# INP-PM/FEDM

Measured on AMD Instinct MI355X. Metric: BDF2 DOF-updates/sec (streamer_discharge 2D axisym), higher is better.
Workload: dtype f64

## Files before the change

### __graft_entry__.py

```python
import os
import subprocess
import sys
from pathlib import Path

ROOT = Path(__file__).resolve().parent
CSRC = ROOT / "fedm_amd" / "csrc"
LIB = ROOT / "fedm_amd" / "libfedm_hip.so"
SOURCES = ["prep.cpp", "kernels.hip", "assemble.hip", "boundary.hip", "spmv.hip", "assemble3.hip", "gd.hip", "gdprep.hip", "amg.hip", "fs_tiles.hip",
           "segregated.hip", "comm.hip", "photo.hip", "diag.hip", "fields.hip", "gd_balance.hip", "gd_fields.hip", "currents.hip", "context.cpp", "photo_abi.cpp", "krylov.cpp", "newton.cpp", "amg_setup.cpp", "hooks.cpp"]
HEADERS = [CSRC / "fedm_internal.hpp", CSRC / "element.hpp", CSRC / "element_lean.hpp", CSRC / "amg.hpp",
           CSRC / "comm.hpp", CSRC / "species_planes.hpp", CSRC / "solver.hpp", CSRC / "device_util.hpp", CSRC / "table_lookup.h", CSRC / "photo.hpp", CSRC / "diag.hpp", CSRC / "fields.hpp", CSRC / "gd_balance.hpp", CSRC / "currents.hpp",
           CSRC / "postproc.hpp", ROOT / "include" / "fedm_hip.h"]


OBJ = CSRC / "_build"
FILE_FLAGS = {"assemble3.hip": ["-mllvm", "-disable-machine-licm"]}


def _stale(lib):
    if not Path(lib).exists():
        return True
    t = Path(lib).stat().st_mtime
    return any(p.stat().st_mtime > t for p in [CSRC / s for s in SOURCES] + HEADERS)


def _compile(hipcc, src, obj, extra):
    cmd = [hipcc, "--offload-arch=gfx950", "-O3", "-std=c++17", "-fPIC", "-c", "-Wno-unused-result",
           "-Wno-unused-value", f"-I{ROOT / 'include'}", f"-I{CSRC}", *FILE_FLAGS.get(Path(src).name, []), *extra,
           "-o", str(obj), str(src)]
    subprocess.run(cmd, check=True)


def build(force=False, lib=LIB, defines=()):
    if force or _stale(lib):
        import fcntl
# ... 101 lines not shown
```

### fedm_amd/_lib.py

```python
import ctypes as C
import os
from pathlib import Path

MAX_SPECIES, MAX_TERMS, MAX_REACTIONS, MAX_TAGS = 4, 6, 8, 8
MAX_QP, MAX_FQP, MAX_EXT_NODES = 32, 8, 10
MAX_TABLES, MAX_TABLE_KNOTS = 16, 4096

EQ_TYPES = {"reaction": 0, "diffusion-reaction": 1, "drift-diffusion-reaction": 2}
BC_KINDS = {"zero flux": 0, "Neumann": 1, "flux source": 2}
DIVERGED = {1: "maximum number of Newton iterations reached",
            2: "NaN or Inf in the residual", 3: "linear solve (GMRES) did not converge"}


class TermSumC(C.Structure):
    _fields_ = [("n_terms", C.c_int32), ("pad_", C.c_int32),
                ("c", C.c_double * MAX_TERMS), ("p", C.c_double * MAX_TERMS),
                ("q", C.c_double * MAX_TERMS), ("r", C.c_double * MAX_TERMS)]


class ModelDesc(C.Structure):
    _fields_ = [
        ("n_species", C.c_int32), ("poisson", C.c_int32), ("axisymmetric", C.c_int32),
        ("n_reactions", C.c_int32),
        ("eq_type", C.c_int32 * MAX_SPECIES), ("Z", C.c_double * MAX_SPECIES),
# ... 57 lines not shown
class MeshDesc(C.Structure):
    _fields_ = [("n_vertices", C.c_int32), ("n_cells", C.c_int32),
                ("coords", C.POINTER(C.c_double)), ("cells", C.POINTER(C.c_int32)),
                ("facet_tags", C.POINTER(C.c_int8)),
                ("n_dirichlet", C.c_int32),
                ("dirichlet_dofs", C.POINTER(C.c_int32)),
                ("dirichlet_vals", C.POINTER(C.c_double)),
                ("n_owned_vertices", C.c_int32),
                ("n_identity_vertices", C.c_int32), ("identity_vertices", C.POINTER(C.c_int32)),
                ("halo_depth", C.c_int32)]


class NewtonOpts(C.Structure):
    _fields_ = [("rtol", C.c_double), ("atol", C.c_double), ("stol", C.c_double),
                ("max_it", C.c_int32), ("ksp_restart", C.c_int32),
                ("ksp_rtol", C.c_double), ("ksp_atol", C.c_double),
                ("ksp_max_it", C.c_int32), ("watch_component", C.c_int32)]


class NewtonReport(C.Structure):
    _fields_ = [("iterations", C.c_int32), ("converged", C.c_int32),
                ("linear_iterations", C.c_int32), ("reason", C.c_int32),
                ("fnorm0", C.c_double), ("fnorm", C.c_double)]


class Csr(C.Structure):
    _fields_ = [("n_rows", C.c_int32), ("n_cols", C.c_int32),
                ("indptr", C.POINTER(C.c_int64)), ("indices", C.POINTER(C.c_int32)),
                ("values", C.POINTER(C.c_double))]


PHOTO_MAX_TERMS = 4


class PhotoDesc(C.Structure):
    _fields_ = [("n_terms", C.c_int32), ("n_src", C.c_int32),
                ("c", C.c_double * PHOTO_MAX_TERMS), ("kappa", C.c_double * PHOTO_MAX_TERMS),
                ("efficiency", C.c_double), ("src_reaction", C.c_int32 * MAX_REACTIONS),
                ("target_species_mask", C.c_uint32), ("zero_tag_mask", C.c_uint32)]


class PhotoHierarchy(C.Structure):
    _fields_ = [("n_levels", C.c_int32), ("nu", C.c_int32),
                ("A", C.POINTER(Csr)), ("P", C.POINTER(Csr)), ("R", C.POINTER(Csr)),
                ("coarse_inverse", C.POINTER(C.c_double)), ("omega", C.c_double)]

# ... 93 lines not shown
    "fedm_debug_gd_reduced_field": (C.c_int, [_P, _D]),
    "fedm_gd_update_mean_energy": (C.c_int, [_P]),
    "fedm_get_state_old": (C.c_int, [_P, _D]),
    "fedm_ctx_destroy": (None, [_P]),
    "fedm_set_state": (C.c_int, [_P, _D, _D, _D]),
    "fedm_get_state": (C.c_int, [_P, _D]),
    "fedm_shift_state": (C.c_int, [_P]),
    "fedm_reset_state": (C.c_int, [_P]),
    "fedm_state_snapshot": (C.c_int, [_P]),
    "fedm_state_restore": (C.c_int, [_P]),
    "fedm_set_step": (C.c_int, [_P, C.c_double, C.c_double]),
    "fedm_set_dirichlet_values": (C.c_int, [_P, _D]),
    "fedm_set_ext_source": (C.c_int, [_P, C.c_int, _D]),
    "fedm_ext_source_program": (C.c_int, [_P, C.c_int, C.c_int, C.POINTER(C.c_int32), C.c_int, _D, C.c_int]),
    "fedm_ext_source_eval": (C.c_int, [_P, C.c_int, _D]),
    "fedm_debug_get_ext_source": (C.c_int, [_P, C.c_int, _D]),
    "fedm_residual": (C.c_int, [_P, _D, _D]),
    "fedm_jacobian": (C.c_int, [_P]),
    "fedm_jacobian_nnz": (C.c_int64, [_P]),
    "fedm_jacobian_csr": (C.c_int, [_P, C.POINTER(C.c_int64), C.POINTER(C.c_int32), _D]),
    "fedm_spmv": (C.c_int, [_P, _D, _D]),
    "fedm_newton_solve": (C.c_int, [_P, C.POINTER(NewtonOpts), C.POINTER(NewtonReport)]),
    "fedm_poisson_solve": (C.c_int, [_P, C.c_double, C.c_int, C.POINTER(C.c_int)]),
    "fedm_poisson_update": (C.c_int, [_P, C.c_double, C.c_int, C.POINTER(C.c_int)]),
    "fedm_newton_solve_species": (C.c_int, [_P, C.POINTER(NewtonOpts), C.POINTER(NewtonReport)]),
    "fedm_segregated_stats": (C.c_int, [_P, C.POINTER(C.c_int64), C.c_int]),
    "fedm_debug_species_assembly": (C.c_int, [_P, C.c_int]),
    "fedm_debug_block_product": (C.c_int, [_P, C.c_int, _D, _D]),
    "fedm_debug_species_linear_solve": (C.c_int, [_P, _D, C.POINTER(NewtonOpts), _D, C.POINTER(C.c_int), _D]),
    "fedm_photo_setup": (C.c_int, [_P, C.POINTER(PhotoDesc), C.POINTER(PhotoHierarchy)]),
    "fedm_photo_update": (C.c_int, [_P, C.c_double, C.c_int, C.POINTER(C.c_int)]),
    "fedm_photo_get": (C.c_int, [_P, _D, _D]),
    "fedm_photo_stats": (C.c_int, [_P, C.POINTER(C.c_int64), C.c_int]),
    "fedm_diag_setup": (C.c_int, [_P, _D, C.POINTER(C.c_int8), C.c_int]),
    "fedm_diagnostics": (C.c_int, [_P, C.POINTER(DiagOpts), C.POINTER(DiagOut)]),
    "fedm_gd_balance_setup": (C.c_int, [_P, _D, C.POINTER(C.c_int8), C.c_int]),
    "fedm_gd_balance": (C.c_int, [_P, C.POINTER(GdBalanceOut)]),
    "fedm_currents_setup": (C.c_int, [_P, C.c_int, _D]),
    "fedm_currents_solve": (C.c_int, [_P, C.POINTER(PhotoHierarchy), _D, C.c_double, C.c_int, C.POINTER(C.c_int)]),
    "fedm_currents_get_psi": (C.c_int, [_P, _D]),
    "fedm_currents": (C.c_int, [_P, C.POINTER(CurrentsOut)]),
    "fedm_fields_setup": (C.c_int, [_P, C.POINTER(Csr)]),
    "fedm_probe_setup": (C.c_int, [_P, C.c_int, C.POINTER(C.c_int32), _D]),
    "fedm_fields": (C.c_int, [_P, C.POINTER(FieldOpts), C.c_int, C.POINTER(FieldReq), _D, _D, C.POINTER(C.c_int32),
                              C.POINTER(C.c_int32)]),
    "fedm_gd_fields_setup": (C.c_int, [_P, C.POINTER(Csr)]),
# ... 109 lines not shown
```

### fedm_amd/cases/streamer.py

```python
from pathlib import Path

import numpy as np

from ..device import DeviceProblem, Model, Reaction
from ..mesh import Marking_boundaries, Mesh, RectangleMesh, geometric_lines
from ..termsum import TermSum, parse

U_W = 18750.0
BOX = 0.0125
BOUNDARIES = [["line", 0.0, 0.0, 0.0, BOX], ["line", BOX, BOX, 0.0, BOX],
              ["line", 0.0, BOX, 0.0, 0.0], ["line", 0.0, BOX, BOX, BOX]]
BC_TYPE = [["zero flux", "Neumann"], ["zero flux", "Neumann"],
           ["zero flux", "zero flux"], ["zero flux", "zero flux"]]
DECK = Path(__file__).resolve().parents[2] / "decks" / "streamer_discharge" / "file_input"
MU_E = "2.3987*E_m**(-0.26)"
D_E = "4.3628e-3*E_m**(0.22)"
ALPHA = "(1.1944e6 + 4.3666e26 * E_m**(-3))*exp(-2.73e7/E_m)-340.75"
N0 = 760.0 * 3.21877e22


def model(mu_e=MU_E, D_e=D_E, alpha=ALPHA, quadrature_degree=2):
    mu = parse(mu_e)
    rate = parse(alpha) * mu * TermSum.field()
    return Model(n_species=2, poisson=True,
# ... 100 lines not shown

SPECIES_NAMES = ("ions", "electrons")

DIAGNOSTIC_COLUMNS = ("t", "z_head", "E_max_axis", "E_max", "N_i", "N_e", "net_charge", "surface_charge_cathode",
                      "surface_charge_anode", "current", "ni_max", "ne_max")


MULTIGRID = dict(nu=1, omega=0.85, hard_poly_degree=2)


def initialise(prob, multigrid=True):
    U = np.zeros((prob.nv, 3))
    U[:, 0], U[:, 1] = initial_log_densities(prob.coords)
    prob.set_state(U, U, U)
    if multigrid:
        prob.setup_multigrid(**MULTIGRID)
        from ..device import chebyshev_weights
        prob.set_fieldsplit(chebyshev_weights(6), hard_weights=chebyshev_weights(4))
    its = prob.poisson_solve(rtol=1e-12)
    U = prob.get_state()
    prob.set_state(U, U, U)
    return U, its



class Stepper:

    partition_name = "single GPU"

    @property
    def assembly_kernel_name(self):
        sz = self.prob.sizes()
        if sz["assembly_variant"] == "lds-patches/one-pass":
            return (f"assemble_lean3_kernel<2,1,{sz['patch_threads']},kept planes> (LDS patches with micro-coloured cell "
                    "order, one pass over the cells, live planes only, F+J)")
        if sz["assembly_variant"] != "lds-patches":
            return f"volume assembly, variant '{sz['assembly_variant']}' (F+J)"
        return (f"assemble_lean2_kernel<2,1,{sz['patch_threads']}> (LDS patches with micro-coloured cell order, one "
                "equation row at a time, F+J)")

    @property
    def multigrid_levels(self):
        return getattr(self.prob, "multigrid_levels", None)

    def __init__(self, prob, dt_init=5e-12, dt_max=5e-12, dt_min=1e-15, ttol=1e-3,
                 relative_tolerance=1e-4, maximum_iterations=20, error_file=None, quiet=True,
                 coupling="coupled"):
        import tempfile
        from .. import functions as ff
        from ..forms import DeviceState, Expression, FunctionAssigner
        self.ff, self.prob = ff, prob
        self.solver = ff.PETScSNESSolver()
        self.solver.parameters["relative_tolerance"] = relative_tolerance
        self.solver.parameters["maximum_iterations"] = maximum_iterations
        self.solver.parameters["coupling"] = coupling
        self.problem = ff.Problem(None, None, [], device_problem=prob)
        self.dt = Expression("time_step", time_step=dt_init, degree=0)
        self.dt_old = Expression("time_step", time_step=1e30, degree=0)
        self.u_new, self.u_old = DeviceState(prob, "new"), DeviceState(prob, "old")
        self.assigner = FunctionAssigner()
        self.error, self.max_error = [0.0] * 2, [1] * 3
        self.ttol, self.dt_min, self.dt_max = ttol, dt_min, dt_max
        if error_file is None:
            error_file = Path(tempfile.mkdtemp(prefix="fedm_amd_")) / "relative error.log"
        self.error_file = Path(error_file)
        open(self.error_file, "w").close()
        self.t, self.steps, self.newton_iterations, self.linear_iterations = 0.0, 0, 0, 0
        self.quiet = quiet
        self.total_dofs = prob.n

    def initialise(self):
        return initialise(self.prob)

    def step(self):
        import contextlib, io
        ff = self.ff
        self.prob.shift_state()
        sink = io.StringIO() if self.quiet else None
        with (contextlib.redirect_stdout(sink) if sink else contextlib.nullcontext()):
            self.t = ff.adaptive_solver(self.solver, self.problem, self.t, self.dt, self.dt_old,
                                        self.u_new, self.u_old, None, None, self.assigner,
                                        self.error, self.error_file, self.max_error, self.ttol,
                                        self.dt_min, time_dependent_arguments=[],
                                        approximation="LFA")
        self.newton_iterations += self.prob.last_report.iterations
        self.linear_iterations += self.prob.last_report.linear_iterations
        self.dt_old.time_step = self.dt.time_step
        self.dt.time_step = ff.adaptive_timestep(self.dt.time_step, self.max_error, self.ttol,
                                                 self.dt_min, self.dt_max)
        self.max_error[2] = self.max_error[1]
        self.max_error[1] = self.max_error[0]
        self.steps += 1
        return self.t

    def diagnose(self):
        if getattr(self, "_diagnose", None) is None:
            self._diagnose = diagnostics(self.prob)
# ... 61 lines not shown
```

### fedm_amd/csrc/context.cpp

```cpp
#include <algorithm>
#include <cmath>
#include <cstdlib>
#include <cstring>

#include "photo.hpp"
#include "solver.hpp"

namespace fedm {

static thread_local std::string g_error;
void set_error(const std::string &msg) { g_error = msg; }

void prof_collect(Ctx &c) {
    Prof &p = c.prof;
    if (p.used == 0) return;
    hipStreamSynchronize(c.stream);
    for (int i = 0; i + 1 < p.used; i += 2) {
        float ms = 0.f;
        if (hipEventElapsedTime(&ms, p.ev[i], p.ev[i + 1]) == hipSuccess) {
            p.ms[p.kind[i / 2]] += ms;
            p.cnt[p.kind[i / 2]]++;
        }
    }
    p.used = 0;
// ... 205 lines not shown
        std::memcpy(buf.data() + sizeof(m) + sizeof(mt), t.x, sizeof(double) * total);
        std::memcpy(buf.data() + sizeof(m) + sizeof(mt) + sizeof(double) * total, t.y, sizeof(double) * total);
    }
    FEDM_HIP_CHECK(hipMalloc((void **)&dst, buf.size()));
    FEDM_HIP_CHECK(hipMemcpy(dst, buf.data(), buf.size(), hipMemcpyHostToDevice));
    return 0;
}

int put_vec(Ctx &c, double *dst, const double *src) {
    if (!src) return 0;
    std::memcpy(c.h_stage, src, sizeof(double) * c.n);
    FEDM_HIP_CHECK(hipMemcpyAsync(dst, c.h_stage, sizeof(double) * c.n, hipMemcpyHostToDevice, c.stream));
    FEDM_HIP_CHECK(hipStreamSynchronize(c.stream));
    return 0;
}

int get_vec(Ctx &c, double *dst, const double *src) {
    FEDM_HIP_CHECK(hipMemcpyAsync(c.h_stage, src, sizeof(double) * c.n, hipMemcpyDeviceToHost, c.stream));
    FEDM_HIP_CHECK(hipStreamSynchronize(c.stream));
    std::memcpy(dst, c.h_stage, sizeof(double) * c.n);
    return 0;
}

}

using namespace fedm;

extern "C" {

const char *fedm_last_error(void) { return g_error.c_str(); }
int fedm_abi_version(void) { return FEDM_ABI_VERSION; }

static int ctx_create_impl(const fedm_mesh_desc *mesh, const fedm_model_desc *model,
                           const fedm_gd_desc *gd, const HostTables &tables, int device, fedm_ctx **out);

static int ctx_create_guarded(const fedm_mesh_desc *mesh, const fedm_model_desc *model,
                              const fedm_gd_desc *gd, const HostTables &tables, int device, fedm_ctx **out) {
    *out = nullptr;
    fedm_ctx *h = nullptr;
    const int rc = ctx_create_impl(mesh, model, gd, tables, device, &h);
    if (rc != 0) {
        const std::string msg = g_error;
        if (h) fedm_ctx_destroy(h);
        g_error = msg;
        return rc;
    }
// ... 467 lines not shown
int fedm_set_state(fedm_ctx *h, const double *u_new, const double *u_old, const double *u_old1) {
    Ctx &c = h->c;
    c.err_cache_comp = -1;
    FEDM_HIP_CHECK(hipSetDevice(c.device));
    if (u_new) c.halo_pending = false;
    if (put_vec(c, c.d_u, u_new) || put_vec(c, c.d_uold, u_old) || put_vec(c, c.d_uold1, u_old1)) return -1;
    return 0;
}

int fedm_get_state(fedm_ctx *h, double *u_new) {
    Ctx &c = h->c;
    FEDM_HIP_CHECK(hipSetDevice(c.device));
    return get_vec(c, u_new, c.d_u);
}

int fedm_get_state_old(fedm_ctx *h, double *u_old) {
    Ctx &c = h->c;
    FEDM_HIP_CHECK(hipSetDevice(c.device));
    return get_vec(c, u_old, c.d_uold);
}

int fedm_shift_state(fedm_ctx *h) {
    Ctx &c = h->c;
    c.err_cache_comp = -1;
    FEDM_HIP_CHECK(hipSetDevice(c.device));
    std::swap(c.d_uold1, c.d_uold);
    launch_scale_copy(c, 1.0, c.d_u, c.d_uold);
    return 0;
}

int fedm_reset_state(fedm_ctx *h) {
    Ctx &c = h->c;
    c.err_cache_comp = -1;
    FEDM_HIP_CHECK(hipSetDevice(c.device));
    launch_scale_copy(c, 1.0, c.d_uold, c.d_u);
    return 0;
}

int fedm_state_snapshot(fedm_ctx *h) {
    Ctx &c = h->c;
    FEDM_HIP_CHECK(hipSetDevice(c.device));
    if (c.halo_pending) {
        comm_halo(c, c.d_u);
        c.halo_pending = false;
    }
    if (!c.d_snapshot) FEDM_HIP_CHECK(hipMalloc((void **)&c.d_snapshot, sizeof(double) * 3 * c.np));
    const double *src[3] = {c.d_u, c.d_uold, c.d_uold1};
    for (int k = 0; k < 3; ++k)
        FEDM_HIP_CHECK(hipMemcpyAsync(c.d_snapshot + (size_t)k * c.np, src[k], sizeof(double) * c.np,
                                      hipMemcpyDeviceToDevice, c.stream));
    FEDM_HIP_CHECK(hipStreamSynchronize(c.stream));
    c.snap_krylov_steps_hint = c.krylov_steps_hint;
    std::copy(std::begin(c.krylov_hints), std::end(c.krylov_hints), std::begin(c.snap_krylov_hints));
    c.snap_newton_its_hint = c.newton_its_hint;
    return 0;
}

int fedm_state_restore(fedm_ctx *h) {
// ... 297 lines not shown
```

### fedm_amd/csrc/newton.cpp

```cpp
#include <chrono>
#include <cmath>

#include "solver.hpp"

namespace fedm {

void set_hard_mode(Ctx &c, bool hard) {
    if (c.fs_alt_active == hard) return;
    c.fs_skip_sample = true;
    hipStreamSynchronize(c.stream);
    iter_graphs_clear(c);
    c.fs_alt_active = hard;
    if (c.fs_alt_sweeps > 0) {
        c.fs_sweeps = hard ? c.fs_alt_sweeps : c.fs_main_sweeps;
        for (int i = 0; i < c.fs_sweeps; ++i) c.fs_w[i] = hard ? c.fs_alt_w[i] : c.fs_main_w[i];
    }
    if (c.amg_alt) std::swap(c.amg, c.amg_alt);
}

static void update_fieldsplit_policy(Ctx &c, int it, int lin_total, int rc,
                                     std::chrono::steady_clock::time_point t_begin) {
    ++c.fs_solves[c.fs_alt_active ? 1 : 0];
    if ((c.fs_alt_sweeps > 0 || c.amg_alt) && it > 0) {
        const double per_solve = (double)lin_total / it;
// ... 149 lines not shown
                    indices[pos] = col * neq + cc;
                    values[pos] = val[(bc * neq2 + cr * neq + cc) * SLICE + l];
                    ++pos;
                }
            }
            indptr[(size_t)v * neq + cr + 1] = pos;
        }
    }
    return 0;
}

int fedm_spmv(fedm_ctx *h, const double *x, double *y) {
    Ctx &c = h->c;
    FEDM_HIP_CHECK(hipSetDevice(c.device));
    FEDM_HIP_CHECK(hipMemsetAsync(c.d_tmp, 0, sizeof(double) * c.np, c.stream));
    if (put_vec(c, c.d_tmp, x)) return -1;
    launch_spmv(c, c.d_tmp, c.d_w, false);
    return get_vec(c, y, c.d_w);
}

int fedm_newton_solve(fedm_ctx *h, const fedm_newton_opts *o, fedm_newton_report *rep) {
    Ctx &c = h->c;
    FEDM_HIP_CHECK(hipSetDevice(c.device));
    c.err_cache_comp = -1;
    const auto t_begin = std::chrono::steady_clock::now();
    int it = 0, lin_total = 0, rc = 0;
    double fnorm = 0.0, fnorm0 = 0.0, snorm = 0.0, xnorm = 0.0;
    while (true) {
        const bool residual_only = it > 0 && it == c.newton_its_hint;
        if (residual_only) {
            launch_assemble(c, false, 0);
            launch_finalize(c, false, 0);
        } else {
            eval_jacobian(c, 0);
        }
        const bool sums_local = c.comm && it > 0 && c.red12_local;
        const bool with_error = residual_only && (!c.comm || sums_local) && o->watch_component > 0 &&
                                o->watch_component <= c.neq;
        if (with_error) launch_field_error_slots34(c, o->watch_component - 1);
        norm2_publish(c, c.d_F, 0, with_error ? 5 : 3, sums_local ? (with_error ? 5 : 3) : 1);
        c.red12_local = false;
        bool planes_done = false;
        if (!residual_only && right_preconditioned(c)) {
            prepare_preconditioner_and_rhs(c);
            planes_done = true;
        }
// ... 45 lines not shown
        }
        if (c.comm && c.assembly_overlap) c.halo_pending = true;
        else comm_halo(c, c.d_u);
        if (comm_failed(c)) {
            rc = -1;
            break;
        }
        ++it;
    }
    if (comm_failed(c)) rc = -1;
    if (rc == 0) c.newton_its_hint = it;
    update_fieldsplit_policy(c, it, lin_total, rc, t_begin);
    write_report(rep, it, lin_total, fnorm0, fnorm, rc);
    if (comm_failed(c)) {
        set_error(c.comm->error);
        return -1;
    }
    if (hipGetLastError() != hipSuccess) {
        set_error("HIP error during Newton solve");
        return -1;
    }
    return rc;
}

int fedm_poisson_solve(fedm_ctx *h, double rtol, int max_it, int *iterations) {
    Ctx &c = h->c;
    c.err_cache_comp = -1;
    FEDM_HIP_CHECK(hipSetDevice(c.device));
    if (!c.poisson) {
        set_error("model has no Poisson row");
        return -2;
    }
    launch_set_dirichlet_state(c);
    launch_assemble(c, true, 1);
    launch_finalize(c, true, 1);
    launch_block_inverse(c);
    launch_scale_copy(c, -1.0, c.d_F, c.d_rhs);
    if (ensure_krylov(c, 1)) return -1;
    const CgResult cg = preconditioned_cg(c, CgMatrix::whole, rtol, max_it);
    launch_axpy(c, 1.0, c.d_V, c.d_u);
    comm_halo(c, c.d_u);
    FEDM_HIP_CHECK(hipStreamSynchronize(c.stream));
    if (iterations) *iterations = cg.it;
    if (comm_failed(c)) {
        set_error(c.comm->error);
        return -1;
// ... 84 lines not shown
    } else {
        launch_assemble(c, false, 0);
        launch_finalize(c, false, 0);
    }
    launch_pick_entries(c, 1, -1.0, c.d_F, c.d_rhs);
    if (ensure_krylov(c, 1)) return -1;
    const CgResult cg = preconditioned_cg(c, CgMatrix::potential_block, rtol, max_it);
    if (std::isfinite(cg.rn)) launch_axpy(c, 1.0, c.d_V, c.d_u);
    FEDM_HIP_CHECK(hipStreamSynchronize(c.stream));
    FEDM_HIP_CHECK(hipGetLastError());
    c.seg_stats[SG_CG_ITS] += cg.it;
    if (iterations) *iterations = cg.it;
    if (!std::isfinite(cg.rn)) return FEDM_DIVERGED_NAN;
    return cg.rn <= rtol * cg.r0 ? 0 : FEDM_DIVERGED_LINEAR;
}

int fedm_field_error(fedm_ctx *h, int component, double *rel_err) {
    Ctx &c = h->c;
    if (component < 0 || component >= c.neq) {
        set_error("component out of range");
        return -2;
    }
    FEDM_HIP_CHECK(hipSetDevice(c.device));
    if (component == c.err_cache_comp) {
        ++c.path_stats[PS_ERR_CACHE_SERVED];
        *rel_err = c.err_cache;
        return 0;
    }
    launch_field_error(c, component);
    read_red(c, 2);
    *rel_err = std::sqrt(c.h_red[0]) / std::sqrt(c.h_red[1]);
    if (comm_failed(c)) {
        set_error(c.comm->error);
        return -1;
    }
    return 0;
}

int fedm_jacobian_poisson_only(fedm_ctx *h) {
    Ctx &c = h->c;
    if (!c.poisson) {
        set_error("model has no Poisson row");
        return -2;
    }
    FEDM_HIP_CHECK(hipSetDevice(c.device));
    launch_set_dirichlet_state(c);
    eval_jacobian(c, 1);
    FEDM_HIP_CHECK(hipStreamSynchronize(c.stream));
    return 0;
}

}
```

### fedm_amd/csrc/solver.hpp

```cpp
#pragma once
#include "amg.hpp"
#include "comm.hpp"
#include "fedm_internal.hpp"

struct fedm_ctx {
    fedm::Ctx c;
};

namespace fedm {

int put_vec(Ctx &c, double *dst, const double *src);
int get_vec(Ctx &c, double *dst, const double *src);

int ensure_krylov(Ctx &c, int restart);
bool right_preconditioned(const Ctx &c);
void prepare_preconditioner_and_rhs(Ctx &c);
void krylov_vector_update(Ctx &c, int k, const double *const *vp, double *w);
void krylov_vector_scale(Ctx &c, double a, const double *x, double *y);
int gmres(Ctx &c, int restart, double rtol, double atol, int max_it, int *its_out, double *rnorm_out,
          const double *bvec, double bscale, double bnorm_known, double *u_update, bool *u_updated,
          int newton_iteration = -1);
int species_gmres(Ctx &c, int restart, double rtol, double atol, int max_it, double bnorm, int *its_out,
                  double *rnorm_out);
enum class CgMatrix { whole, potential_block };
struct CgResult {
    int it;
    double r0, rn;
};
CgResult preconditioned_cg(Ctx &c, CgMatrix matrix, double rtol, int max_it);

int build_amg(Ctx &c, int n_first_rows, int n_levels, const fedm_csr *A, const fedm_csr *P, const fedm_csr *R,
              const double *coarse_inverse, int nu, double omega, Amg **out, int composite_from,
              const double *poly_w = nullptr );

void set_hard_mode(Ctx &c, bool hard);
int segregated_refusal(Ctx &c, const char *who, bool species);
int ensure_seg_dinv(Ctx &c);
enum SegStat { SG_UPDATES = 0, SG_CG_ITS, SG_SOLVES, SG_ONE_PASS, SG_FALLBACK, SG_NEWTON_ITS, SG_KRYLOV_STEPS };

}
```

### fedm_amd/device.py

```python
import ctypes as C
import os
from dataclasses import dataclass, field
from typing import List, Optional, Sequence, Tuple

import numpy as np

from . import _lib, quadrature
from .photo import Photoionization
from .physical_constants import elementary_charge, epsilon_0
from .termsum import TermSum


@dataclass
class Reaction:
    k: TermSum
    power: Sequence[int]
    net: Sequence[int]


@dataclass
class Walls:
    vth: Sequence[Sequence[float]]
    ref: Sequence[Sequence[float]]
    gamma: Sequence[float]
# ... 472 lines not shown
    order = locality_order(coords, cells) if reorder else np.arange(coords.shape[0])
    inv = np.empty(coords.shape[0], dtype=np.int64)
    inv[order] = np.arange(coords.shape[0])
    cdev = np.ascontiguousarray(coords[order])
    kdev = np.ascontiguousarray(inv[cells], dtype=np.int32)
    mesh = _lib.MeshDesc()
    mesh.n_vertices, mesh.n_cells = coords.shape[0], cells.shape[0]
    mesh.coords = _dp(cdev)
    mesh.cells = kdev.ctypes.data_as(C.POINTER(C.c_int32))
    out = (C.c_int64 * 10)()
    rc = lib.fedm_fieldsplit_tiles_stats(C.byref(mesh), int(slices_per_tile), int(layers), out)
    if rc != 0:
        raise RuntimeError(f"fedm_fieldsplit_tiles_stats failed ({rc}): {_lib.last_error()}")
    keys = ("n_tiles", "row_width", "max_vertices", "max_rows", "total_rows", "total_vertices", "bytes", "violations",
            "lds_bytes_species_kernel", "lds_bytes_multigrid_kernel")
    return dict(zip(keys, (int(v) for v in out)))


SOLVER_PATH_STATS = ("cycles", "steps_single", "steps_pair", "steps_last", "steps_dropped", "updates_made_up",
                     "second_passes", "fused_updates", "generic_updates", "deferred_norm", "nothing_to_solve",
                     "residual_only_right", "residual_only_wrong", "err_cache_served", "steps_used", "steps_ahead",
                     "steps_ahead_later", "solves", "breakdowns", "exhausted", "newton_max_it", "verified",
                     "verify_failed", "second_passes_device")

_VARIANTS = ("global colouring", "lds-patches/unrolled", "lds-patches", "lds-patches/one-pass",
             "lmea/dual-number colours", "lmea/atomics", "lmea/element buffer, cell order",
             "lmea/element buffer, destination order", "lmea/element buffer, destination order, columns side by side")


class DeviceProblem:

    def __init__(self, coords, cells, model: Model, facet_tags=None,
                 dirichlet_dofs=(), dirichlet_vals=(), device=0, reorder=True, n_owned=None,
                 identity_vertices=None, halo_depth=1):
        self.lib = _lib.load()
        self.model = model
        self.coords = np.ascontiguousarray(coords, dtype=np.float64)
        self.cells = np.ascontiguousarray(cells, dtype=np.int32)
        self.nv, self.nc = self.coords.shape[0], self.cells.shape[0]
        if self.coords.ndim != 2 or self.coords.shape[1] != 2 or self.cells.ndim != 2 or self.cells.shape[1] != 3:
            raise ValueError("DeviceProblem: coords must be (n_vertices, 2) and cells (n_cells, 3)")
        if self.nc and (self.cells.min() < 0 or self.cells.max() >= self.nv):
            raise ValueError("DeviceProblem: cell vertex index out of range")
        self.n_eq = model.n_eq
        self.n = self.nv * self.n_eq
        self._tags = None if facet_tags is None else np.ascontiguousarray(facet_tags, dtype=np.int8)
# ... 780 lines not shown
    def fieldsplit_policy(self):
        out = (C.c_int64 * 4)()
        self._check(self.lib.fedm_fieldsplit_policy(self._h, out), "fedm_fieldsplit_policy")
        return dict(policy="measured (wall time per Newton iteration)" if out[0] else "Krylov counts",
                    alternative_active=bool(out[1]), solves_main_set=int(out[2]), solves_alternative_set=int(out[3]))

    def clear_multigrid(self):
        self.lib.fedm_amg_clear(self._h)

    def newton_solve(self, rtol=1e-9, max_it=50, atol=1e-10, stol=1e-16,
                     ksp_restart=30, ksp_rtol=1e-5, ksp_atol=1e-50, ksp_max_it=10000):
        watch = getattr(self, "watch_component", None)
        o = _lib.NewtonOpts(rtol, atol, stol, max_it, ksp_restart, ksp_rtol, ksp_atol, ksp_max_it,
                            0 if watch is None else int(watch) + 1)
        r = _lib.NewtonReport()
        if self._photo_stale:
            self.photo_update()
        rc = self.lib.fedm_newton_solve(self._h, C.byref(o), C.byref(r))
        self.last_report = NewtonReport(r.iterations, bool(r.converged), r.linear_iterations,
                                        r.fnorm0, r.fnorm)
        self._check(rc, "fedm_newton_solve")
        return r.iterations, True

    def poisson_solve(self, rtol=1e-10, max_it=20000):
        its = C.c_int()
        self._check(self.lib.fedm_poisson_solve(self._h, float(rtol), int(max_it), C.byref(its)),
                    "fedm_poisson_solve")
        return its.value

    def poisson_update(self, rtol=1e-10, max_it=20000):
        its = C.c_int()
        rc = self.lib.fedm_poisson_update(self._h, float(rtol), int(max_it), C.byref(its))
        self.last_poisson_iterations = its.value
        self._check(rc, "fedm_poisson_update")
        return its.value

    def newton_solve_species(self, rtol=1e-9, max_it=50, atol=1e-10, stol=1e-16,
                             ksp_restart=30, ksp_rtol=1e-5, ksp_atol=1e-50, ksp_max_it=10000):
        o = _lib.NewtonOpts(rtol, atol, stol, max_it, ksp_restart, ksp_rtol, ksp_atol, ksp_max_it, 0)
        r = _lib.NewtonReport()
        rc = self.lib.fedm_newton_solve_species(self._h, C.byref(o), C.byref(r))
        self.last_report = NewtonReport(r.iterations, bool(r.converged), r.linear_iterations,
                                        r.fnorm0, r.fnorm)
        self._check(rc, "fedm_newton_solve_species")
        return r.iterations, True

# ... 234 lines not shown
```

### include/fedm_hip.h

```cpp
#ifndef FEDM_HIP_H
#define FEDM_HIP_H

#include <stdint.h>

#ifdef __cplusplus
extern "C" {
#endif

#define FEDM_MAX_SPECIES 4
#define FEDM_MAX_TERMS 6
#define FEDM_MAX_REACTIONS 8
#define FEDM_MAX_TAGS 8
#define FEDM_MAX_QP 32
#define FEDM_MAX_FQP 8
#define FEDM_MAX_EXT_NODES 10
#define FEDM_MAX_TABLES 16
#define FEDM_MAX_TABLE_KNOTS 4096

#define FEDM_EQ_REACTION 0
#define FEDM_EQ_DIFFUSION_REACTION 1
#define FEDM_EQ_DRIFT_DIFFUSION_REACTION 2

#define FEDM_BC_ZERO_FLUX 0
#define FEDM_BC_NEUMANN 1
// ... 169 lines not shown
#define FEDM_EXPR_MAX_PARAMS 16
#define FEDM_EXPR_STACK 24
enum {
    FEDM_OP_CONST = 0,
    FEDM_OP_X = 1,
    FEDM_OP_PARAM = 2,
    FEDM_OP_ADD = 3, FEDM_OP_SUB = 4, FEDM_OP_MUL = 5, FEDM_OP_DIV = 6, FEDM_OP_POW = 7,
    FEDM_OP_NEG = 8, FEDM_OP_EXP = 9, FEDM_OP_LOG = 10, FEDM_OP_SQRT = 11, FEDM_OP_SIN = 12, FEDM_OP_COS = 13,
    FEDM_OP_TAN = 14, FEDM_OP_FABS = 15, FEDM_OP_TANH = 16, FEDM_OP_ATAN = 17
};
int fedm_ext_source_program(fedm_ctx *ctx, int species, int n_ops, const int32_t *ops ,
                            int n_consts, const double *consts, int n_params);
int fedm_ext_source_eval(fedm_ctx *ctx, int species, const double *params );
int fedm_debug_get_ext_source(fedm_ctx *ctx, int species, double *out );

int fedm_residual(fedm_ctx *ctx, double *F_out , double *fnorm );
int fedm_jacobian(fedm_ctx *ctx);
int64_t fedm_jacobian_nnz(fedm_ctx *ctx);
int fedm_jacobian_csr(fedm_ctx *ctx, int64_t *indptr, int32_t *indices, double *values);
int fedm_spmv(fedm_ctx *ctx, const double *x, double *y);

int fedm_newton_solve(fedm_ctx *ctx, const fedm_newton_opts *opts, fedm_newton_report *rep);
int fedm_poisson_solve(fedm_ctx *ctx, double rtol, int max_it, int *iterations);


int fedm_poisson_update(fedm_ctx *ctx, double rtol, int max_it, int *iterations);
int fedm_newton_solve_species(fedm_ctx *ctx, const fedm_newton_opts *opts, fedm_newton_report *rep);
int fedm_segregated_stats(fedm_ctx *ctx, int64_t out[8], int reset);
int fedm_debug_species_assembly(fedm_ctx *ctx, int jacobian);
int fedm_debug_block_product(fedm_ctx *ctx, int which, const double *x, double *y);
int fedm_debug_species_linear_solve(fedm_ctx *ctx, const double *b, const fedm_newton_opts *opts, double *x, int *its,
                                    double *rnorm);

typedef struct {
    int32_t n_terms;
    int32_t n_src;
    double c[4];
    double kappa[4];
    double efficiency;
    int32_t src_reaction[FEDM_MAX_REACTIONS];
    uint32_t target_species_mask;
    uint32_t zero_tag_mask;
} fedm_photo_desc;
typedef struct {
    int32_t n_levels, nu;
    const fedm_csr *A, *P, *R;
// ... 214 lines not shown
```

Before: 255.6 million.

## Move the BDF2 adaptive time-step loop into a single native C call

Adds fedm_bdf2_step, which runs state shift, Newton solve, field-error estimate, rejection/retry and the PID step controller in C++. The Python Stepper uses it by default for plain coupled single-GPU setups, caching ctypes structs and error-log formatting. This is meant to cut the Python and ctypes overhead of several calls per step. In exchange it duplicates controller logic in C, which must match the Python version bit for bit (hence libm pow via a volatile pointer).

```diff
diff --git a/__graft_entry__.py b/__graft_entry__.py
--- a/__graft_entry__.py
+++ b/__graft_entry__.py
@@ -7,10 +7,10 @@
 CSRC = ROOT / "fedm_amd" / "csrc"
 LIB = ROOT / "fedm_amd" / "libfedm_hip.so"
 SOURCES = ["prep.cpp", "kernels.hip", "assemble.hip", "boundary.hip", "spmv.hip", "assemble3.hip", "gd.hip", "gdprep.hip", "amg.hip", "fs_tiles.hip",
-           "segregated.hip", "comm.hip", "photo.hip", "diag.hip", "fields.hip", "gd_balance.hip", "gd_fields.hip", "currents.hip", "context.cpp", "photo_abi.cpp", "krylov.cpp", "newton.cpp", "amg_setup.cpp", "hooks.cpp"]
+           "segregated.hip", "comm.hip", "photo.hip", "diag.hip", "fields.hip", "gd_balance.hip", "gd_fields.hip", "currents.hip", "context.cpp", "photo_abi.cpp", "krylov.cpp", "newton.cpp", "timestep.cpp", "amg_setup.cpp", "hooks.cpp"]
 HEADERS = [CSRC / "fedm_internal.hpp", CSRC / "element.hpp", CSRC / "element_lean.hpp", CSRC / "amg.hpp",
            CSRC / "comm.hpp", CSRC / "species_planes.hpp", CSRC / "solver.hpp", CSRC / "device_util.hpp", CSRC / "table_lookup.h", CSRC / "photo.hpp", CSRC / "diag.hpp", CSRC / "fields.hpp", CSRC / "gd_balance.hpp", CSRC / "currents.hpp",
-           CSRC / "postproc.hpp", ROOT / "include" / "fedm_hip.h"]
+           CSRC / "postproc.hpp", CSRC / "step_controller.hpp", ROOT / "include" / "fedm_hip.h"]
 
 
 OBJ = CSRC / "_build"
diff --git a/fedm_amd/_lib.py b/fedm_amd/_lib.py
--- a/fedm_amd/_lib.py
+++ b/fedm_amd/_lib.py
@@ -103,6 +103,28 @@
     _fields_ = [("iterations", C.c_int32), ("converged", C.c_int32),
                 ("linear_iterations", C.c_int32), ("reason", C.c_int32),
                 ("fnorm0", C.c_double), ("fnorm", C.c_double)]
+
+
+class StepOpts(C.Structure):
+    _fields_ = [("newton", NewtonOpts), ("t", C.c_double), ("dt", C.c_double), ("dt_old", C.c_double),
+                ("error", C.c_double * 3), ("max_error", C.c_double * 3),
+                ("ttol", C.c_double), ("dt_min", C.c_double), ("dt_max", C.c_double), ("tol", C.c_double),
+                ("n_error", C.c_int32), ("coupling", C.c_int32), ("krylov_scaling", C.c_int32), ("pad_", C.c_int32)]
+
+
+class StepAttempt(C.Structure):
+    _fields_ = [("error", C.c_double), ("dt_old", C.c_double), ("step", C.c_double),
+                ("newton_code", C.c_int32), ("accepted", C.c_int32)]
+
+
+class StepReport(C.Structure):
+    _fields_ = [("t", C.c_double), ("dt", C.c_double), ("dt_old", C.c_double),
+                ("error", C.c_double * 3), ("max_error", C.c_double * 3),
+                ("attempts", C.c_int32), ("newton_iterations", C.c_int32), ("linear_iterations", C.c_int32),
+                ("pad_", C.c_int32), ("last", NewtonReport)]
+
+
+STEP_DT_MIN = 16
 
 
 class Csr(C.Structure):
@@ -242,6 +264,8 @@
     "fedm_spmv": (C.c_int, [_P, _D, _D]),
     "fedm_newton_solve": (C.c_int, [_P, C.POINTER(NewtonOpts), C.POINTER(NewtonReport)]),
     "fedm_poisson_solve": (C.c_int, [_P, C.c_double, C.c_int, C.POINTER(C.c_int)]),
+    "fedm_bdf2_step": (C.c_int, [_P, C.POINTER(StepOpts), C.POINTER(StepReport), C.POINTER(StepAttempt), C.c_int]),
+    "fedm_debug_step_controller": (C.c_int, [C.c_double] * 7 + [_D]),
     "fedm_poisson_update": (C.c_int, [_P, C.c_double, C.c_int, C.POINTER(C.c_int)]),
     "fedm_newton_solve_species": (C.c_int, [_P, C.POINTER(NewtonOpts), C.POINTER(NewtonReport)]),
     "fedm_segregated_stats": (C.c_int, [_P, C.POINTER(C.c_int64), C.c_int]),
diff --git a/fedm_amd/cases/streamer.py b/fedm_amd/cases/streamer.py
--- a/fedm_amd/cases/streamer.py
+++ b/fedm_amd/cases/streamer.py
@@ -1,3 +1,4 @@
+import os
 from pathlib import Path
 
 import numpy as np
@@ -146,6 +147,8 @@
     prob.set_state(U, U, U)
     return U, its
 
+
+_STEP_CALLS = frozenset(("shift_state", "set_step", "newton_solve", "field_error", "reset_state"))
 
 
 class Stepper:
@@ -192,11 +195,73 @@
         self.t, self.steps, self.newton_iterations, self.linear_iterations = 0.0, 0, 0, 0
         self.quiet = quiet
         self.total_dofs = prob.n
+        self.native_step = os.environ.get("FEDM_NATIVE_STEP", "1") != "0"
 
     def initialise(self):
         return initialise(self.prob)
 
+    def _plain_setup(self):
+        prob = self.prob
+        return (self.solver.parameters.get("coupling", "coupled") == "coupled" and self.problem.before_solve is None
+                and type(prob) is DeviceProblem and not prob._has_photo() and prob.n_owned == prob.nv
+                and not hasattr(prob, "_plan_keep")
+                and prob.__dict__.keys().isdisjoint(_STEP_CALLS))
+
+    def _step_native(self):
+        p, prob, error, max_error, dt, dt_old = self.solver.parameters, self.prob, self.error, self.max_error, self.dt, self.dt_old
+        key = (p["relative_tolerance"], p["maximum_iterations"], p["absolute_tolerance"], p["solution_tolerance"],
+               p["krylov_restart"], p["krylov_relative_tolerance"], p["krylov_maximum_iterations"],
+               p.get("krylov_residual_scaling", "none"), self.ttol, self.dt_min, self.dt_max, len(error))
+        if key != getattr(prob, "_step_key", None):
+            if key[7] not in ("none", "rows"):
+                raise ValueError(f"krylov_residual_scaling must be 'none' or 'rows', got {key[7]!r}")
+            prob.step_setup(self.ttol, self.dt_min, self.dt_max, n_error=len(error), rtol=key[0], max_it=key[1],
+                            atol=key[2], stol=key[3], ksp_restart=key[4], ksp_rtol=key[5], ksp_max_it=key[6],
+                            krylov_scaling=key[7], key=key)
+        step, step_old = dt.time_step, dt_old.time_step
+        rc, v, n = prob.bdf2_step(self.t, step, step_old, error, max_error)
+        rows = self.__dict__.get("_rows")
+        if rows is None or rows.closed or self._rows_of != self.error_file:
+            rows, self._rows_of = self.ff._error_log(self.error_file), self.error_file
+            self._rows = rows
+        if n[0] == 1:
+            if n[7] == 0:
+                text = self.__dict__.setdefault("_row_text", {})
+                a, b = text.get(step_old), text.get(step)
+                if a is None or b is None:
+                    if len(text) > 8:
+                        text.clear()
+                    a, b = text[step_old], text[step] = f"{step_old:<23}", f"{step:<23}"
+                rows.write(f"{v[3]:<23}  {a}  {b}\n")
+        else:
+            attempts = prob.step_attempts()
+            for a_error, a_dt_old, a_step, code, _ in attempts:
+                if code == 0:
+                    rows.write(f"{a_error:<23}  {a_dt_old:<23}  {a_step:<23}\n")
+            if n[0] > len(attempts):
+                import warnings
+                warnings.warn(f"step {self.steps}: {n[0]} attempts, the error log has the first {len(attempts)}")
+        rows.flush()
+        if not self.quiet:
+            for a_error, _, a_step, code, accepted in prob.step_attempts():
+                print(f"Attempted to solve the equation for t = {self.t} with dt = {a_step}: "
+                      + ("accepted" if accepted else "error above the tolerance, repeated with a smaller time step"
+                         if code == 0 else "the solver failed, repeated with half the time step"), flush=True)
+        error[0] = v[3]
+        max_error[0], max_error[1], max_error[2] = v[6], v[7], v[8]
+        dt.time_step = v[1]
+        if rc:
+            raise SystemExit("Minimum time-step size reached, program is terminating.")
+        self.t = t = v[0]
+        dt_old.time_step = v[2]
+        self.newton_iterations += n[4]
+        self.linear_iterations += n[6]
+        self.steps += 1
+        return t
+
     def step(self):
+        if self.native_step and self._plain_setup():
+            return self._step_native()
         import contextlib, io
         ff = self.ff
         self.prob.shift_state()
diff --git a/fedm_amd/csrc/context.cpp b/fedm_amd/csrc/context.cpp
--- a/fedm_amd/csrc/context.cpp
+++ b/fedm_amd/csrc/context.cpp
@@ -251,6 +251,17 @@
     return 0;
 }
 
+void shift_state(Ctx &c) {
+    c.err_cache_comp = -1;
+    std::swap(c.d_uold1, c.d_uold);
+    launch_scale_copy(c, 1.0, c.d_u, c.d_uold);
+}
+
+void reset_state(Ctx &c) {
+    c.err_cache_comp = -1;
+    launch_scale_copy(c, 1.0, c.d_uold, c.d_u);
+}
+
 }
 
 using namespace fedm;
@@ -764,18 +775,15 @@
 
 int fedm_shift_state(fedm_ctx *h) {
     Ctx &c = h->c;
-    c.err_cache_comp = -1;
-    FEDM_HIP_CHECK(hipSetDevice(c.device));
-    std::swap(c.d_uold1, c.d_uold);
-    launch_scale_copy(c, 1.0, c.d_u, c.d_uold);
+    FEDM_HIP_CHECK(hipSetDevice(c.device));
+    shift_state(c);
     return 0;
 }
 
 int fedm_reset_state(fedm_ctx *h) {
     Ctx &c = h->c;
-    c.err_cache_comp = -1;
-    FEDM_HIP_CHECK(hipSetDevice(c.device));
-    launch_scale_copy(c, 1.0, c.d_uold, c.d_u);
+    FEDM_HIP_CHECK(hipSetDevice(c.device));
+    reset_state(c);
     return 0;
 }
 
diff --git a/fedm_amd/csrc/newton.cpp b/fedm_amd/csrc/newton.cpp
--- a/fedm_amd/csrc/newton.cpp
+++ b/fedm_amd/csrc/newton.cpp
@@ -195,6 +195,14 @@
 int fedm_newton_solve(fedm_ctx *h, const fedm_newton_opts *o, fedm_newton_report *rep) {
     Ctx &c = h->c;
     FEDM_HIP_CHECK(hipSetDevice(c.device));
+    return newton_loop(c, o, rep);
+}
+
+}
+
+namespace fedm {
+
+int newton_loop(Ctx &c, const fedm_newton_opts *o, fedm_newton_report *rep) {
     c.err_cache_comp = -1;
     const auto t_begin = std::chrono::steady_clock::now();
     int it = 0, lin_total = 0, rc = 0;
@@ -286,6 +294,26 @@
     }
     return rc;
 }
+
+int field_error(Ctx &c, int component, double *rel_err) {
+    if (component == c.err_cache_comp) {
+        ++c.path_stats[PS_ERR_CACHE_SERVED];
+        *rel_err = c.err_cache;
+        return 0;
+    }
+    launch_field_error(c, component);
+    read_red(c, 2);
+    *rel_err = std::sqrt(c.h_red[0]) / std::sqrt(c.h_red[1]);
+    if (comm_failed(c)) {
+        set_error(c.comm->error);
+        return -1;
+    }
+    return 0;
+}
+
+}
+
+extern "C" {
 
 int fedm_poisson_solve(fedm_ctx *h, double rtol, int max_it, int *iterations) {
     Ctx &c = h->c;
@@ -416,19 +444,7 @@
         return -2;
     }
     FEDM_HIP_CHECK(hipSetDevice(c.device));
-    if (component == c.err_cache_comp) {
-        ++c.path_stats[PS_ERR_CACHE_SERVED];
-        *rel_err = c.err_cache;
-        return 0;
-    }
-    launch_field_error(c, component);
-    read_red(c, 2);
-    *rel_err = std::sqrt(c.h_red[0]) / std::sqrt(c.h_red[1]);
-    if (comm_failed(c)) {
-        set_error(c.comm->error);
-        return -1;
-    }
-    return 0;
+    return field_error(c, component, rel_err);
 }
 
 int fedm_jacobian_poisson_only(fedm_ctx *h) {
diff --git a/fedm_amd/csrc/solver.hpp b/fedm_amd/csrc/solver.hpp
--- a/fedm_amd/csrc/solver.hpp
+++ b/fedm_amd/csrc/solver.hpp
@@ -11,6 +11,8 @@
 
 int put_vec(Ctx &c, double *dst, const double *src);
 int get_vec(Ctx &c, double *dst, const double *src);
+void shift_state(Ctx &c);
+void reset_state(Ctx &c);
 
 int ensure_krylov(Ctx &c, int restart);
 bool right_preconditioned(const Ctx &c);
@@ -33,6 +35,8 @@
               const double *coarse_inverse, int nu, double omega, Amg **out, int composite_from,
               const double *poly_w = nullptr );
 
+int newton_loop(Ctx &c, const fedm_newton_opts *o, fedm_newton_report *rep);
+int field_error(Ctx &c, int component, double *rel_err);
 void set_hard_mode(Ctx &c, bool hard);
 int segregated_refusal(Ctx &c, const char *who, bool species);
 int ensure_seg_dinv(Ctx &c);
diff --git a/fedm_amd/csrc/step_controller.hpp b/fedm_amd/csrc/step_controller.hpp
--- /dev/null
+++ b/fedm_amd/csrc/step_controller.hpp
@@ -0,0 +1,40 @@
+#pragma once
+#include <cmath>
+
+namespace fedm {
+
+inline double libm_pow(double x, double y) {
+    static double (*volatile fn)(double, double) = std::pow;
+    return fn(x, y);
+}
+
+inline double step_within(double dt, double dt_min, double dt_max) {
+    const double m = dt_max < dt ? dt_max : dt;
+    return dt_min > m ? dt_min : m;
+}
+
+inline double step_controller(double dt, double e0, double e1, double e2, double tol, double dt_min, double dt_max) {
+    const double proportional = libm_pow(e1 / e0, 0.075);
+    const double integral = libm_pow(tol / e0, 0.175);
+    const double derivative = libm_pow(libm_pow(e1, 2.0) / (e0 * e2), 0.01);
+    const double factor = proportional * integral * derivative;
+    return step_within(dt * factor, dt_min, dt_max);
+}
+
+inline double step_max_error(const double *error, int n) {
+    double m = error[0];
+    for (int i = 1; i < n; ++i)
+        if (error[i] > m) m = error[i];
+    return m;
+}
+
+inline double step_rejected_dt(double dt, bool solver_failed, double ttol, double max_error0) {
+    return solver_failed ? dt * 0.5 : dt * (0.5 * ttol / max_error0);
+}
+
+inline double step_back(double t, double step) {
+    const double advanced = t + step;
+    return advanced - step;
+}
+
+}
diff --git a/fedm_amd/csrc/timestep.cpp b/fedm_amd/csrc/timestep.cpp
--- /dev/null
+++ b/fedm_amd/csrc/timestep.cpp
@@ -0,0 +1,123 @@
+#include "solver.hpp"
+#include "step_controller.hpp"
+
+using namespace fedm;
+
+static int step_refusal(Ctx &c, const fedm_step_opts *o) {
+    const char *who = "fedm_bdf2_step: ";
+    if (c.model_kind != 0) {
+        set_error(std::string(who) + "the LMEA family refreshes its coefficient fields between the shift and the solve "
+                  "(LFA models only)");
+        return -2;
+    }
+    if (c.comm || c.n_owned != c.nv) {
+        set_error(std::string(who) + "one GPU only (this context has a transport or ghost vertices): every rank has to "
+                  "take the same decision from all-reduced sums");
+        return -2;
+    }
+    if (o->coupling != 0) {
+        set_error(std::string(who) + "the coupled step only (the segregated one is fedm_poisson_update followed by "
+                  "fedm_newton_solve_species)");
+        return -2;
+    }
+    if (c.photo) {
+        set_error(std::string(who) + "this context has photoionisation set up, whose source is refreshed between the "
+                  "shift and the solve (fedm_photo_update)");
+        return -2;
+    }
+    if (o->newton.watch_component < 1 || o->newton.watch_component > c.neq) {
+        set_error(std::string(who) + "newton.watch_component must name the component whose change is the step's error "
+                  "(1 + its index)");
+        return -2;
+    }
+    if (o->n_error < 1 || o->n_error > 3) {
+        set_error(std::string(who) + "n_error must be 1, 2 or 3");
+        return -2;
+    }
+    if (o->krylov_scaling != 0 && o->krylov_scaling != 1) {
+        set_error(std::string(who) + "krylov scaling mode must be 0 (none) or 1 (rows)");
+        return -2;
+    }
+    return 0;
+}
+
+extern "C" {
+
+int fedm_bdf2_step(fedm_ctx *h, const fedm_step_opts *o, fedm_step_report *rep, fedm_step_attempt *records,
+                   int capacity) {
+    if (!h || !o || !rep) {
+        set_error("fedm_bdf2_step: null argument");
+        return -2;
+    }
+    Ctx &c = h->c;
+    if (const int refused = step_refusal(c, o)) return refused;
+    FEDM_HIP_CHECK(hipSetDevice(c.device));
+    if (c.krylov_scaling != o->krylov_scaling)
+        if (const int rc = fedm_set_krylov_scaling(h, o->krylov_scaling)) return rc;
+    const int watched = o->newton.watch_component - 1;
+    fedm_step_report r{};
+    double t = o->t, dt = o->dt;
+    const double dt_old = o->dt_old;
+    for (int i = 0; i < 3; ++i) {
+        r.error[i] = o->error[i];
+        r.max_error[i] = o->max_error[i];
+    }
+    const auto record = [&](double error, double step, int code, bool accepted) {
+        if (records && r.attempts < capacity) records[r.attempts] = {error, dt_old, step, code, accepted ? 1 : 0};
+        ++r.attempts;
+    };
+    const auto finish = [&](int rc) {
+        r.t = t;
+        *rep = r;
+        return rc;
+    };
+    shift_state(c);
+    while (true) {
+        const double step = dt;
+        c.dt = step;
+        c.dt_old = dt_old;
+        const int nrc = newton_loop(c, &o->newton, &r.last);
+        r.newton_iterations += r.last.iterations;
+        r.linear_iterations += r.last.linear_iterations;
+        if (nrc < 0) {
+            r.dt = dt;
+            r.dt_old = dt_old;
+            return finish(-1);
+        }
+        bool accepted = false;
+        if (nrc == 0) {
+            if (field_error(c, watched, &r.error[0])) return finish(-1);
+            r.max_error[0] = step_max_error(r.error, o->n_error);
+            accepted = !(r.error[0] >= o->ttol);
+            record(r.error[0], step, 0, accepted);
+        } else {
+            record(0.0, step, nrc, false);
+        }
+        if (accepted) {
+            t = t + step;
+            break;
+        }
+        t = step_back(t, step);
+        dt = step_rejected_dt(dt, nrc != 0, o->ttol, r.max_error[0]);
+        reset_state(c);
+        if (dt < o->dt_min) {
+            r.dt = dt;
+            r.dt_old = dt_old;
+            return finish(FEDM_STEP_DT_MIN);
+        }
+    }
+    r.dt_old = dt;
+    r.dt = step_controller(dt, r.max_error[0], r.max_error[1], r.max_error[2], o->tol, o->dt_min, o->dt_max);
+    r.max_error[2] = r.max_error[1];
+    r.max_error[1] = r.max_error[0];
+    return finish(0);
+}
+
+int fedm_debug_step_controller(double dt, double e0, double e1, double e2, double tol, double dt_min, double dt_max,
+                               double *out) {
+    if (!out) return -2;
+    *out = step_controller(dt, e0, e1, e2, tol, dt_min, dt_max);
+    return 0;
+}
+
+}
diff --git a/fedm_amd/device.py b/fedm_amd/device.py
--- a/fedm_amd/device.py
+++ b/fedm_amd/device.py
@@ -1,5 +1,6 @@
 import ctypes as C
 import os
+import struct
 from dataclasses import dataclass, field
 from typing import List, Optional, Sequence, Tuple
 
@@ -518,6 +519,12 @@
                      "residual_only_right", "residual_only_wrong", "err_cache_served", "steps_used", "steps_ahead",
                      "steps_ahead_later", "solves", "breakdowns", "exhausted", "newton_max_it", "verified",
                      "verify_failed", "second_passes_device")
+
+_STEP_IN, _STEP_COUNTS = struct.Struct("9d"), struct.Struct("8i")
+_STEP_IN_AT, _STEP_COUNTS_AT = _lib.StepOpts.t.offset, _lib.StepReport.attempts.offset
+_STEP_PAD = (0.0, 0.0, 0.0)
+assert _lib.StepOpts.max_error.offset == _STEP_IN_AT + 48 and _lib.StepReport.max_error.offset == 48
+assert _lib.StepReport.last.offset == _STEP_COUNTS_AT + 16 and _lib.NewtonReport.fnorm0.offset == 16
 
 _VARIANTS = ("global colouring", "lds-patches/unrolled", "lds-patches", "lds-patches/one-pass",
              "lmea/dual-number colours", "lmea/atomics", "lmea/element buffer, cell order",
@@ -1344,6 +1351,62 @@
         self._check(rc, "fedm_newton_solve")
         return r.iterations, True
 
+    STEP_RECORDS = 16
+
+    def step_setup(self, ttol, dt_min, dt_max, tol=None, watch=None, n_error=2, rtol=1e-9, max_it=50, atol=1e-10,
+                   stol=1e-16, ksp_restart=30, ksp_rtol=1e-5, ksp_atol=1e-50, ksp_max_it=10000, krylov_scaling="none",
+                   coupling="coupled", key=None):
+        self._step_key = key
+        if getattr(self, "_step_call", None) is None:
+            o, r, rec = _lib.StepOpts(), _lib.StepReport(), (_lib.StepAttempt * self.STEP_RECORDS)()
+            self._step_call = (o, r, rec, C.byref(o), C.byref(r), self.lib.fedm_bdf2_step, self._h)
+        o = self._step_call[0]
+        n = o.newton
+        n.rtol, n.atol, n.stol, n.max_it = rtol, atol, stol, max_it
+        n.ksp_restart, n.ksp_rtol, n.ksp_atol, n.ksp_max_it = ksp_restart, ksp_rtol, ksp_atol, ksp_max_it
+        self.watch_component = self.n_eq - 2 if watch is None else int(watch)
+        n.watch_component = self.watch_component + 1
+        if not 1 <= n_error <= 3:
+            raise ValueError("step_setup: the error list has one to three entries")
+        o.n_error = n_error
+        o.ttol, o.dt_min, o.dt_max, o.tol = ttol, dt_min, dt_max, ttol if tol is None else tol
+        o.coupling = 0 if coupling == "coupled" else 1
+        o.krylov_scaling = ("none", "rows").index(krylov_scaling)
+
+    def bdf2_step(self, t, dt, dt_old, error, max_error, **setup):
+        if setup:
+            self.step_setup(**setup)
+        o, r, rec, o_ref, r_ref, call, h = self._step_call
+        _STEP_IN.pack_into(o, _STEP_IN_AT, t, dt, dt_old, *error, *_STEP_PAD[len(error):], *max_error)
+        rc = call(h, o_ref, r_ref, rec, self.STEP_RECORDS)
+        if rc != 0 and rc != _lib.STEP_DT_MIN:
+            self._check(rc, "fedm_bdf2_step")
+        self._last_report = None
+        return rc, _STEP_IN.unpack_from(r, 0), _STEP_COUNTS.unpack_from(r, _STEP_COUNTS_AT)
+
+    @property
+    def step_report(self):
+        return self._step_call[1]
+
+    def step_attempts(self):
+        r, rec = self._step_call[1], self._step_call[2]
+        return [(a.error, a.dt_old, a.step, a.newton_code, bool(a.accepted)) for a in rec[:min(r.attempts, self.STEP_RECORDS)]]
+
+    @property
+    def last_report(self):
+        rep = self.__dict__.get("_last_report")
+        if rep is None:
+            if self.__dict__.get("_step_call") is None:
+                raise AttributeError("last_report: no solve has run")
+            last = self._step_call[1].last
+            rep = self._last_report = NewtonReport(last.iterations, bool(last.converged), last.linear_iterations,
+                                                   last.fnorm0, last.fnorm)
+        return rep
+
+    @last_report.setter
+    def last_report(self, rep):
+        self._last_report = rep
+
     def poisson_solve(self, rtol=1e-10, max_it=20000):
         its = C.c_int()
         self._check(self.lib.fedm_poisson_solve(self._h, float(rtol), int(max_it), C.byref(its)),
diff --git a/include/fedm_hip.h b/include/fedm_hip.h
--- a/include/fedm_hip.h
+++ b/include/fedm_hip.h
@@ -215,6 +215,41 @@
 
 int fedm_newton_solve(fedm_ctx *ctx, const fedm_newton_opts *opts, fedm_newton_report *rep);
 int fedm_poisson_solve(fedm_ctx *ctx, double rtol, int max_it, int *iterations);
+
+typedef struct {
+    fedm_newton_opts newton;
+    double t, dt, dt_old;
+    double error[3];
+    double max_error[3];
+    double ttol, dt_min, dt_max;
+    double tol;
+    int32_t n_error;
+    int32_t coupling;
+    int32_t krylov_scaling;
+    int32_t pad_;
+} fedm_step_opts;
+
+typedef struct {
+    double error, dt_old, step;
+    int32_t newton_code;
+    int32_t accepted;
+} fedm_step_attempt;
+
+typedef struct {
+    double t;
+    double dt, dt_old;
+    double error[3], max_error[3];
+    int32_t attempts;
+    int32_t newton_iterations, linear_iterations;
+    int32_t pad_;
+    fedm_newton_report last;
+} fedm_step_report;
+
+#define FEDM_STEP_DT_MIN 16
+int fedm_bdf2_step(fedm_ctx *ctx, const fedm_step_opts *opts, fedm_step_report *rep, fedm_step_attempt *records,
+                   int capacity);
+int fedm_debug_step_controller(double dt, double e0, double e1, double e2, double tol, double dt_min, double dt_max,
+                               double *out);
 
 
 int fedm_poisson_update(fedm_ctx *ctx, double rtol, int max_it, int *iterations);
```

Result: no change. 255.0 million (-0.2%).
